# Anaesthesiaye/sound_event_detection_transformer

Hardware: AMD Instinct MI355X
Metric: audio clips/sec training throughput (B=64, 10s@64-mel) (higher is better)
Workload: dtype bf16

## Files before the change

include/sedt_hip.h:

```cpp
#ifndef SEDT_HIP_H
#define SEDT_HIP_H
#include <stddef.h>
#include <stdint.h>

#ifdef __cplusplus
extern "C" {
#endif

#define SEDT_F32 0
#define SEDT_BF16 1
#define SEDT_BF16X3 2
#define SEDT_I16 3

#define SEDT_ACT_NONE 0
#define SEDT_ACT_RELU 1
#define SEDT_ACT_SIGMOID 2

const char* sedt_last_error(void);
int sedt_version(void);

typedef struct SedtIgemm {
  int32_t M, N, K;
  const void* A;
  const void* B;
// ... 64 lines not shown
int sedt_split3(const SedtSplitJob* jobs, int njobs, void* stream);

#define SEDT_MAX_REDUCE_JOBS 40
typedef struct SedtReduceJob {
  const float* slab;
  const float* rowscale;
  float* out;
  const float* colsum_slab;
  float* bias_out;
  int32_t splitk, R, taps, Ci;
  int32_t blk0;
  int32_t cs_splitk;
} SedtReduceJob;
int sedt_multi_wgrad_reduce(const SedtReduceJob* jobs, int njobs, const SedtPrefetch* pf, void* stream);

int sedt_skinny_linear_fwd(const void* x, int64_t ldx, const float* w, const float* bias, void* y, int64_t ldy, int M, int N,
                           int K, int act, int out_f32, int dtype, void* stream);
size_t sedt_skinny_linear_bwd_scratch(int K);
int sedt_skinny_linear_bwd(const float* g, const float* ysaved, int64_t ldg, const float* w, const void* x, int64_t ldx,
                           const void* mask, int64_t ldm, void* gx, int64_t ldo, float* dw, float* db, float* scratch, int M, int N,
                           int K, int act, int accumulate_gx, int dtype, void* stream);

int sedt_colsum(const void* in, int64_t ld, int rows, int cols, int in_f32, int dtype, float* out,
                float* scratch, size_t scratch_bytes, void* stream);
size_t sedt_colsum_scratch(int rows, int cols);
int sedt_dropout_grad(const void* in, int64_t ldi, void* out, int64_t ldo, int rows, int cols, float p,
                      uint32_t seed, const uint32_t* seed_ptr, int dtype, void* stream);
int sedt_add(const void* a, const void* b, void* out, int rows, int cols, int b_mod, int dtype, void* stream);
int sedt_add_n(const void* const* srcs, int n, void* out, int64_t numel, int dtype, void* stream);
int sedt_cast(const void* in, int in_dtype, void* out, int out_dtype, int64_t n, void* stream);
// ... 323 lines not shown
```

sound_event_detection_transformer_amd/csrc/host.cpp:

```cpp
#include <math.h>
#include <stdint.h>
#include <vector>
#include "../../include/sedt_hip.h"

namespace sedt { void set_error(const char* fmt, ...); }

template <typename F>
static void lsa_rows_le_cols(int n, int m, F a, std::vector<int>& row_of_col) {
  const double INF = 1e300;
  std::vector<double> u(n + 1, 0.0), v(m + 1, 0.0), minv(m + 1);
  std::vector<int> p(m + 1, 0), way(m + 1, 0);
  std::vector<char> used(m + 1);
  for (int i = 1; i <= n; ++i) {
    p[0] = i;
    int j0 = 0;
    std::fill(minv.begin(), minv.end(), INF);
    std::fill(used.begin(), used.end(), 0);
    do {
      used[j0] = 1;
      int i0 = p[j0], j1 = 0;
      double delta = INF;
      for (int j = 1; j <= m; ++j) {
        if (used[j]) continue;
        double cur = a(i0 - 1, j - 1) - u[i0] - v[j];
// ... 53 lines not shown
extern "C" int sedt_sizeof(int which) {
  switch (which) {
    case 0: return (int)sizeof(SedtIgemm);
    case 1: return (int)sizeof(SedtReduceJob);
    case 2: return (int)sizeof(SedtSplitJob);
    case 3: return (int)sizeof(SedtPrefetch);
    case 4: return (int)sizeof(SedtCriterion);
    case 5: return (int)sizeof(SedtMatch);
    case 6: return (int)sizeof(SedtChunk);
    case 7: return (int)sizeof(SedtBnJob);
    case 8: return (int)sizeof(SedtPackJob);
    case 9: return (int)sizeof(SedtFragJob);
    case 10: return (int)sizeof(SedtPoolAt);
    case 11: return (int)sizeof(SedtCopyJob);
    case 12: return (int)sizeof(SedtViewAug);
    default: return -1;
  }
}
```

sound_event_detection_transformer_amd/csrc/igemm.hip:

```cpp
#include <stdlib.h>
#include "common.h"

namespace sedt {

template <typename T> struct Cfg;
template <> struct Cfg<float> {
  static constexpr int BK = 32, PITCH = 33, EPC = 4, KSTEP = 2, UK = 1;
};
template <> struct Cfg<bf16_t> {
  static constexpr int BK = 64, PITCH = 72, EPC = 8, KSTEP = 16, UK = 4;
};

struct GatherGeom {
  int Hi, Wi, Ci, Ho, Wo, KH, KW, sh, sw, ph, pw, dh, dw, transposed;
};

__device__ __forceinline__ long gather_pix(const GatherGeom& g, int n, int ho, int wo, int kh, int kw) {
  int hi, wi;
  if (!g.transposed) {
    hi = ho * g.sh - g.ph + kh * g.dh;
    wi = wo * g.sw - g.pw + kw * g.dw;
    if ((unsigned)hi >= (unsigned)g.Hi || (unsigned)wi >= (unsigned)g.Wi) return -1;
  } else {
    int th = ho + g.ph - kh * g.dh, tw = wo + g.pw - kw * g.dw;
// ... 627 lines not shown
    long a, b;
    if (wgrad_lds_envelope(*args, &a, &b) == 0) {
      snprintf(out, cap, "%s", wgrad4_ok(*args) ? "wgrad4_group_kernel" : "wgrad3_group_kernel");
      return 0;
    }
  }
  describe.on = true;
  describe.name[0] = 0;
  const int r = sedt_igemm(args, dtype, nullptr);
  describe.on = false;
  if (r == 0) snprintf(out, cap, "%s", describe.name);
  return r;
}

namespace sedt {
int wgrad3_group_try(const SedtIgemm* jobs, int njobs, hipStream_t st);
bool wgrad4_shape_ok(int M, int N);
int wgrad4_tile_m(int M, int N);
int igemm3_group_try(const SedtIgemm* jobs, int njobs, hipStream_t st);
}

extern "C" int sedt_igemm_group(const SedtIgemm* jobs, int njobs, int dtype, void* stream) {
  SEDT_REQUIRE(jobs && njobs >= 1, "igemm_group: bad arguments");
  for (int i = 0; i < njobs; ++i)
    if (int r = check_rmap(jobs[i])) return r;
  if (dtype == SEDT_BF16 && njobs >= 2) {
    const int r = sedt::igemm3_group_try(jobs, njobs, reinterpret_cast<hipStream_t>(stream));
    if (r >= 0) return r;
  }
  for (int i = 0; i < njobs; ++i)
    if (int r = sedt_igemm(&jobs[i], dtype, stream)) return r;
// ... 5 lines not shown
  SEDT_REQUIRE(jobs && njobs >= 1 && out && cap > 0, "igemm_group_describe: bad arguments");
  out[0] = 0;
  if (dtype != SEDT_BF16 || njobs < 2) return 0;
  describe.on = true;
  describe.name[0] = 0;
  const int r = igemm3_group_try(jobs, njobs, nullptr);
  describe.on = false;
  if (r == 0) snprintf(out, cap, "%s", describe.name);
  return r > 0 ? r : 0;
}

extern "C" int sedt_wgrad_group(const SedtIgemm* jobs, int njobs, int dtype, void* stream) {
  SEDT_REQUIRE(jobs && njobs >= 1, "wgrad_group: bad arguments");
  for (int i = 0; i < njobs; ++i) SEDT_REQUIRE(!jobs[i].rmap, "wgrad_group: a weight-gradient problem takes no residual map (job %d)", i);
  if (dtype == SEDT_BF16) {
    const int r = sedt::wgrad3_group_try(jobs, njobs, reinterpret_cast<hipStream_t>(stream));
    if (r >= 0) return r;
  }
  for (int i = 0; i < njobs; ++i)
    if (int r = sedt_igemm(&jobs[i], dtype, stream)) return r;
  return 0;
}

#include "wgrad3_body.h"
namespace sedt {
int wgrad3_group_build(const SedtIgemm* jobs, int njobs, WgradGroup* g);
extern thread_local const WgradGroup* co_group;
extern thread_local bool co_taken;
}

extern "C" int sedt_igemm_co(const SedtIgemm* main, const SedtIgemm* wjobs, int nw, int dtype, void* stream, int* taken) {
  using namespace sedt;
  SEDT_REQUIRE(main && (nw == 0 || wjobs) && taken, "igemm_co: bad arguments");
  *taken = 0;
  for (int i = 0; i < nw; ++i) SEDT_REQUIRE(!wjobs[i].rmap, "igemm_co: a weight-gradient rider takes no residual map (job %d)", i);
// ... 61 lines not shown
```

sound_event_detection_transformer_amd/csrc/wgrad3.hip:

```cpp
#include <stdlib.h>
#include <algorithm>
#include "wgrad3_body.h"

namespace sedt {

template <int BN>
__global__ __launch_bounds__(256) void wgrad3_kernel(const SedtIgemm p, const unsigned a_bytes, const unsigned b_bytes,
                                                     const int nmajor) {
  wgrad3_body<BN>(p, a_bytes, b_bytes, nmajor, blockIdx.x, blockIdx.y);
}

__global__ __launch_bounds__(256) void wgrad3_group_kernel(const WgradGroup g) { wgrad_group_run(g, blockIdx.x); }

template <int BN>
static int launch_wgrad3(const SedtIgemm& p, unsigned a_bytes, unsigned b_bytes, hipStream_t st) {
  SEDT_DESCRIBE("wgrad3_kernel<%d>", BN);
  constexpr size_t lds = (size_t)2 * (64 * ROWB + 64 * BN * 2);
  static bool attr_set = false;
  auto kern = wgrad3_kernel<BN>;
  if (!attr_set) {
    hipError_t e = hipFuncSetAttribute(reinterpret_cast<const void*>(kern), hipFuncAttributeMaxDynamicSharedMemorySize, (int)lds);
    if (e != hipSuccess) {
      set_error("wgrad3: hipFuncSetAttribute failed: %s", hipGetErrorString(e));
      return 1;
// ... 6 lines not shown
    const char* e = sedt::dev_getenv("SEDT_WGRAD_NMAJOR");
    force = e ? atoi(e) : -1;
  }
  const int nmajor = force >= 0 ? force : (p.N > p.M ? 1 : 0);
  hipLaunchKernelGGL(kern, dim3(nwg, p.splitk > 1 ? p.splitk : 1), dim3(256), lds, st, p, a_bytes, b_bytes, nmajor);
  return check_launch("wgrad3");
}

static bool wgrad3_conv_ok(const SedtIgemm& p) {
  return !(p.conv && ((64 % p.Wo) != 0 || p.Ho * p.Wo < 64 || p.Ho < 64 / p.Wo));
}

int wgrad_lds_envelope(const SedtIgemm& p, long* a_bytes, long* b_bytes);
bool wgrad4_ok(const SedtIgemm& p);
int launch_wgrad4(const SedtIgemm& p, unsigned a_bytes, unsigned b_bytes, hipStream_t st);
int launch_wgrad4_group(WgradGroup& g, hipStream_t st);

int wgrad3_group_try(const SedtIgemm* jobs, int njobs, hipStream_t st) {
  static int on = -1;
  if (on < 0) {
    const char* e = sedt::dev_getenv("SEDT_WGRAD_GROUP");
    on = (e && e[0] == '0') ? 0 : 1;
  }
  if (!on || njobs < 1) return -1;
  long ab[WG_MAXG], bb[WG_MAXG];
  for (int base = 0; base < njobs; base += WG_MAXG) {
    const int n = std::min(WG_MAXG, njobs - base);
    for (int i = 0; i < n; ++i) {
      const SedtIgemm& p = jobs[base + i];
      if (!p.trans || wgrad_lds_envelope(p, &ab[i], &bb[i]) != 0 || !wgrad3_conv_ok(p)) return -1;
    }
  }
  static bool attr_set = false;
  constexpr size_t lds = (size_t)2 * (64 * ROWB + 64 * 64 * 2);
  if (!attr_set) {
    hipError_t e = hipFuncSetAttribute(reinterpret_cast<const void*>(wgrad3_group_kernel), hipFuncAttributeMaxDynamicSharedMemorySize,
                                       (int)lds);
    if (e != hipSuccess) {
      set_error("wgrad3 group: hipFuncSetAttribute failed: %s", hipGetErrorString(e));
      return 1;
    }
    attr_set = true;
  }
  for (int base = 0; base < njobs; base += WG_MAXG) {
    WgradGroup g, gw;
    g.n = gw.n = 0;
    const int n = std::min(WG_MAXG, njobs - base);
    int blk = 0;
    for (int j = 0; j < n; ++j) {
      const SedtIgemm& p = jobs[base + j];
      long a, b;
      wgrad_lds_envelope(p, &a, &b);
      if (wgrad4_ok(p)) {
        const int i = gw.n++;
        gw.p[i] = p;
        gw.a_bytes[i] = (unsigned)a;
        gw.b_bytes[i] = (unsigned)b;
        continue;
      }
      const int i = g.n++;
      g.p[i] = p;
      g.a_bytes[i] = (unsigned)a;
      g.b_bytes[i] = (unsigned)b;
      g.nwg[i] = ((p.N + 63) / 64) * ((p.M + 63) / 64);
      g.nmajor[i] = (p.N > p.M ? 1 : 0) + ((p.splitk >= 8 && p.splitk % 8 == 0) ? 2 : 0);
      g.blk0[i] = blk;
      blk += (g.nwg[i] * (p.splitk > 1 ? p.splitk : 1) + 7) / 8 * 8;
    }
    if (gw.n > 0)
      if (int r = launch_wgrad4_group(gw, st)) return r;
    if (g.n > 0) {
      g.blk0[g.n] = blk;
      hipLaunchKernelGGL(wgrad3_group_kernel, dim3(blk), dim3(256), lds, st, g);
      if (int r = check_launch("wgrad3_group")) return r;
    }
  }
  return 0;
}

int wgrad3_group_build(const SedtIgemm* jobs, int njobs, WgradGroup* g) {
  if (njobs < 1 || njobs > WG_MAXG) return -1;
  g->n = njobs;
  int blk = 0;
  for (int i = 0; i < njobs; ++i) {
    const SedtIgemm& p = jobs[i];
// ... 62 lines not shown
```

sound_event_detection_transformer_amd/csrc/wgrad3_body.h:

```cpp
#pragma once
#include "lds_gemm_common.h"

namespace sedt {

typedef __attribute__((ext_vector_type(4))) short w3_s16x4;
typedef __attribute__((ext_vector_type(8))) short w3_s16x8;
typedef __attribute__((address_space(3))) w3_s16x4 w3_lds_s16x4;

__device__ __forceinline__ int w3_uniform(int v) { return __builtin_amdgcn_readfirstlane(v); }

__device__ __forceinline__ int w3_swz(int row) {
  const int v = (row >> 1) & 7;
  return ((v & 1) << 2) | (v & 2) | (v >> 2);
}

template <int BN, bool CONV>
__device__ __forceinline__ void wgrad3_impl(const SedtIgemm& p, const unsigned a_bytes, const unsigned b_bytes, const int nmajor,
                                            const int bx, const int by) {
  constexpr int BM = 64, BKP = 64;
  constexpr int NI = BN / 64;
  constexpr int A_BYTES = BKP * ROWB;
  constexpr int B_ROWB = BN * 2;
  constexpr int STAGE_BYTES = A_BYTES + BKP * B_ROWB;
  constexpr int GA = 2, GB = BN / 32;
// ... 216 lines not shown
  else wgrad3_impl<BN, false>(p, a_bytes, b_bytes, nmajor, bx, by);
}

constexpr int WG_MAXG = 10;
struct WgradGroup {
  int n;
  int blk0[WG_MAXG + 1];
  int nwg[WG_MAXG];
  int nmajor[WG_MAXG];
  unsigned a_bytes[WG_MAXG], b_bytes[WG_MAXG];
  SedtIgemm p[WG_MAXG];
};

static_assert(sizeof(WgradGroup) <= 3900, "WgradGroup must fit the 4 KB kernel-argument segment");

__device__ __forceinline__ void wgrad_group_run(const WgradGroup& g, const int b) {
  int i = 0;
  while (i + 1 < g.n && b >= g.blk0[i + 1]) ++i;
  const int local = b - g.blk0[i];
  const int nwg = g.nwg[i], sk = g.p[i].splitk > 1 ? g.p[i].splitk : 1;
  if (local >= nwg * sk) return;
  if (g.nmajor[i] >= 2) {
    const int j = local >> 3;
    wgrad3_body<64>(g.p[i], g.a_bytes[i], g.b_bytes[i], g.nmajor[i], j % nwg, (local & 7) + 8 * (j / nwg));
  } else {
    wgrad3_body<64>(g.p[i], g.a_bytes[i], g.b_bytes[i], g.nmajor[i], local % nwg, local / nwg);
  }
}

}
// ... 1 lines not shown
```

sound_event_detection_transformer_amd/csrc/wgrad4.hip:

```cpp
#include <stdlib.h>
#include <algorithm>
#include "wgrad3_body.h"

namespace sedt {

__device__ __forceinline__ int w4_swz(int row) { return (row & 3) << 2; }

template <bool CONV, int S, int NA>
__device__ __forceinline__ void wgrad4_impl(const SedtIgemm& p, const unsigned a_bytes, const unsigned b_bytes, const int nmajor,
                                            const int bx, const int by) {
  constexpr int BM = 128 * NA, BN = 128, BKP = 64, NW = 8;
  constexpr int IMG_ROWB = 256;
  constexpr int IMG_BYTES = BKP * IMG_ROWB;
  constexpr int STAGE_BYTES = (NA + 1) * IMG_BYTES;
  constexpr int B_IMG = NA * IMG_BYTES;
  constexpr int CPR = 16, RPI = 4;
  constexpr int GB = BKP / RPI / NW, GA = NA * GB;
  constexpr int G = GA + GB;
  constexpr int MI = 2 * NA;
  constexpr unsigned OOB = 0x80000000u;
  extern __shared__ __attribute__((aligned(16))) unsigned char smem[];
  const int t = threadIdx.x, lane = t & 63;
  const int wave = w3_uniform(t >> 6);
  const int kgrp = wave >> 2;
  const int wm = ((wave & 3) >> 1) * (32 * MI), wn = (wave & 1) * 64;
// ... 246 lines not shown
        }
  }
  __syncthreads();
  if (kgrp == 1) {
#pragma unroll
    for (int i = 0; i < MI; ++i)
#pragma unroll
      for (int j = 0; j < 2; ++j)
#pragma unroll
        for (int r = 0; r < 16; ++r) {
          const int row = wm + i * 32 + (r & 3) + 8 * (r >> 2) + 4 * fhalf;
          Cs[row * CP + wn + j * 32 + frow] += acc[i][j][r];
        }
  }
  __syncthreads();
  float* out = p.splitk > 1 ? p.slab + (long)by * p.M * p.N : reinterpret_cast<float*>(p.C);
  const long ldo = p.splitk > 1 ? p.N : p.ldc;
#pragma unroll
  for (int c = 0; c < BM * (BN / 4) / (NW * 64); ++c) {
    const int u = t + c * NW * 64;
    const int trow = u / (BN / 4), cc = (u % (BN / 4)) * 4;
    *reinterpret_cast<float4*>(out + (long)(m0 + trow) * ldo + n0 + cc) = *reinterpret_cast<const float4*>(Cs + trow * CP + cc);
  }
}

template <int S>
__device__ __forceinline__ void wgrad4_body(const SedtIgemm& p, const unsigned a_bytes, const unsigned b_bytes, const int nmajor,
                                            const int bx, const int by) {
  if (nmajor & 2) {
    if (p.conv) wgrad4_impl<true, 3, 2>(p, a_bytes, b_bytes, nmajor, bx, by);
    else wgrad4_impl<false, 3, 2>(p, a_bytes, b_bytes, nmajor, bx, by);
    return;
  }
  if (p.conv) wgrad4_impl<true, S, 1>(p, a_bytes, b_bytes, nmajor, bx, by);
  else wgrad4_impl<false, S, 1>(p, a_bytes, b_bytes, nmajor, bx, by);
}

template <int S>
__global__ __launch_bounds__(512) void wgrad4_kernel(const SedtIgemm p, const unsigned a_bytes, const unsigned b_bytes,
                                                     const int nmajor) {
  wgrad4_body<S>(p, a_bytes, b_bytes, nmajor, blockIdx.x, blockIdx.y);
}

template <int S>
__global__ __launch_bounds__(512) void wgrad4_group_kernel(const WgradGroup g) {
  const int b = blockIdx.x;
  int i = 0;
  while (i + 1 < g.n && b >= g.blk0[i + 1]) ++i;
  const int local = b - g.blk0[i];
  const int nwg = g.nwg[i], sk = g.p[i].splitk > 1 ? g.p[i].splitk : 1;
  if (local >= nwg * sk) return;
  wgrad4_body<S>(g.p[i], g.a_bytes[i], g.b_bytes[i], g.nmajor[i], local % nwg, local / nwg);
}

static int wg4_stages() {
  static int s = -1;
  if (s < 0) {
    const char* e = sedt::dev_getenv("SEDT_WGRAD4_STAGES");
    s = (e && atoi(e) == 3) ? 3 : (e && atoi(e) == 4) ? 4 : 3;
  }
  return s;
}
int wgrad4_tile_m(int M, int N) {
  static int bm = -1, min_tiles = 1;
  if (bm < 0) {
    const char* e = sedt::dev_getenv("SEDT_WGRAD4_BM");
    bm = (e && atoi(e) == 128) ? 128 : 256;
// ... 55 lines not shown
  SEDT_DESCRIBE("wgrad4_kernel<%d>", wg4_stages());
  static bool attr_set = false;
  if (!attr_set) {
    if (wg4_attr(wgrad4_kernel<3>, "wgrad4") || wg4_attr(wgrad4_kernel<4>, "wgrad4")) return 1;
    attr_set = true;
  }
  const int bm = wgrad4_tile_m(p.M, p.N);
  const int nwg = (p.N / 128) * (p.M / bm);
  const int nmajor = (p.N > p.M ? 1 : 0) | (bm == 256 ? 2 : 0);
  const dim3 grid(nwg, p.splitk > 1 ? p.splitk : 1);
  if (wg4_stages() == 4) hipLaunchKernelGGL(wgrad4_kernel<4>, grid, dim3(512), wg4_lds(), st, p, a_bytes, b_bytes, nmajor);
  else hipLaunchKernelGGL(wgrad4_kernel<3>, grid, dim3(512), wg4_lds(), st, p, a_bytes, b_bytes, nmajor);
  return check_launch("wgrad4");
}

int launch_wgrad4_group(WgradGroup& g, hipStream_t st) {
  static bool attr_set = false;
  if (!attr_set) {
    if (wg4_attr(wgrad4_group_kernel<3>, "wgrad4 group") || wg4_attr(wgrad4_group_kernel<4>, "wgrad4 group")) return 1;
    attr_set = true;
  }
  int blk = 0;
  for (int i = 0; i < g.n; ++i) {
    const SedtIgemm& p = g.p[i];
    const int bm = wgrad4_tile_m(p.M, p.N);
    g.nwg[i] = (p.N / 128) * (p.M / bm);
    g.nmajor[i] = (p.N > p.M ? 1 : 0) | (bm == 256 ? 2 : 0) | (wg4_cbmajor(p) ? 4 : 0);
    g.blk0[i] = blk;
    blk += (g.nwg[i] * (p.splitk > 1 ? p.splitk : 1) + 7) / 8 * 8;
  }
  g.blk0[g.n] = blk;
  if (wg4_stages() == 4) hipLaunchKernelGGL(wgrad4_group_kernel<4>, dim3(blk), dim3(512), wg4_lds(), st, g);
  else hipLaunchKernelGGL(wgrad4_group_kernel<3>, dim3(blk), dim3(512), wg4_lds(), st, g);
  return check_launch("wgrad4_group");
}

}
```

sound_event_detection_transformer_amd/lib.py:

```python
import ctypes as C
import os

import torch

HERE = os.path.dirname(os.path.abspath(__file__))
LIB_PATH = os.path.join(HERE, 'libsedt_hip.so')
if os.environ.get('SEDT_LIB_AB') and os.environ.get('SEDT_DEV') == '1':
    LIB_PATH = os.environ['SEDT_LIB_AB']

F32, BF16 = 0, 1
BF16X3 = 2
I16 = 3
GEMM_X3 = False


def gemm_dtype(dtype):
    return BF16X3 if (dtype == F32 and GEMM_X3) else dtype
ACT_NONE, ACT_RELU, ACT_SIGMOID = 0, 1, 2
TORCH_DTYPE = {F32: torch.float32, BF16: torch.bfloat16}


class SedtIgemm(C.Structure):
    _fields_ = [
        ('M', C.c_int32), ('N', C.c_int32), ('K', C.c_int32),
# ... 12 lines not shown
        ('splitk', C.c_int32), ('slab', C.c_void_p),
        ('tile_m', C.c_int32), ('tile_n', C.c_int32),
        ('colsum_out', C.c_void_p),
        ('bits_out', C.c_void_p), ('ldbits', C.c_int64), ('mask_bits', C.c_int32), ('f32ep', C.c_int32),
        ('omap', C.c_int32), ('o_Hi', C.c_int32), ('o_Wi', C.c_int32), ('o_sh', C.c_int32), ('o_sw', C.c_int32), ('o_h0', C.c_int32),
        ('o_w0', C.c_int32), ('btap_on', C.c_int32), ('btap', C.c_int32 * 8), ('split_out', C.c_void_p), ('awrap', C.c_int32), ('rmap', C.c_int32), ('bfrag', C.c_void_p),
    ]


class SedtReduceJob(C.Structure):
    _fields_ = [('slab', C.c_void_p), ('rowscale', C.c_void_p), ('out', C.c_void_p), ('colsum_slab', C.c_void_p),
                ('bias_out', C.c_void_p), ('splitk', C.c_int32), ('R', C.c_int32), ('taps', C.c_int32), ('Ci', C.c_int32),
                ('blk0', C.c_int32), ('cs_splitk', C.c_int32)]


CRIT_MAXL = 8


class SedtCriterion(C.Structure):
    _fields_ = [(n, C.c_void_p) for n in ('logits', 'boxes', 'at', 'tc', 'coef', 'wbox', 'tbox', 'gt_weak', 'tgt_len',
                                           'num_boxes', 'empty_weight', 'dlogits', 'dboxes', 'dboxes2', 'dat', 'out')] + \
               [(n, C.c_int32) for n in ('L', 'B', 'ns', 'Q', 'C', 'n_lab', 'Bat')] + \
               [('layer_of', C.c_int32 * CRIT_MAXL), ('w_ce', C.c_float * CRIT_MAXL), ('w_bbox', C.c_float * CRIT_MAXL),
                ('w_giou', C.c_float * CRIT_MAXL), ('w_weak', C.c_float), ('fl', C.c_int32), ('alpha_fl', C.c_float),
                ('gamma_fl', C.c_float), ('nonfinite', C.c_void_p), ('split', C.c_void_p), ('Qs', C.c_int32), ('q0', C.c_int32),
                ('total', C.c_void_p), ('at_p', C.c_void_p), ('dat_p', C.c_void_p), ('w_weak_p', C.c_float), ('wp_all', C.c_int32),
                ('Bp', C.c_int32)]


class SedtPoolAt(C.Structure):
# ... 36 lines not shown
    for i, t in enumerate(ts):
        a.ptr[i], a.bytes[i] = t.data_ptr(), t.numel() * t.element_size()
    return C.byref(a)


MAX_REDUCE_JOBS = 40
_vp, _i, _i64, _f, _d, _u32, _sz = C.c_void_p, C.c_int, C.c_int64, C.c_float, C.c_double, C.c_uint32, C.c_size_t

SIGNATURES = {
    'sedt_last_error': (C.c_char_p, []),
    'sedt_version': (_i, []),
    'sedt_sizeof': (_i, [_i]),
    'sedt_igemm': (_i, [C.POINTER(SedtIgemm), _i, _vp]),
    'sedt_igemm_group': (_i, [C.POINTER(SedtIgemm), _i, _i, _vp]),
    'sedt_wgrad_group': (_i, [C.POINTER(SedtIgemm), _i, _i, _vp]),
    'sedt_igemm_co': (_i, [C.POINTER(SedtIgemm), C.POINTER(SedtIgemm), _i, _i, _vp, C.POINTER(C.c_int)]),
    'sedt_igemm_splitk': (_i, [_i, _i, _i, _i]),
    'sedt_igemm_describe': (_i, [C.POINTER(SedtIgemm), _i, _i, C.c_char_p, _i]),
    'sedt_igemm_group_describe': (_i, [C.POINTER(SedtIgemm), _i, _i, C.c_char_p, _i]),
    'sedt_wgrad_reduce': (_i, [_vp, _i, _i, _i, _i, _vp, _vp, _vp]),
    'sedt_wgrad_reduce_bias': (_i, [_vp, _i, _i, _i, _i, _vp, _vp, _vp, _vp, _vp]),
    'sedt_split3': (_i, [C.POINTER(SedtSplitJob), _i, _vp]),
    'sedt_copy2d': (_i, [C.POINTER(SedtCopyJob), _i, _vp]),
    'sedt_multi_wgrad_reduce': (_i, [C.POINTER(SedtReduceJob), _i, C.POINTER(SedtPrefetch), _vp]),
    'sedt_skinny_linear_fwd': (_i, [_vp, _i64, _vp, _vp, _vp, _i64, _i, _i, _i, _i, _i, _i, _vp]),
    'sedt_skinny_linear_bwd_scratch': (_sz, [_i]),
    'sedt_skinny_linear_bwd': (_i, [_vp, _vp, _i64, _vp, _vp, _i64, _vp, _i64, _vp, _i64, _vp, _vp, _vp, _i, _i, _i, _i, _i, _i, _vp]),
    'sedt_colsum': (_i, [_vp, _i64, _i, _i, _i, _i, _vp, _vp, _sz, _vp]),
    'sedt_colsum_scratch': (_sz, [_i, _i]),
    'sedt_dropout_grad': (_i, [_vp, _i64, _vp, _i64, _i, _i, _f, _u32, _vp, _i, _vp]),
# ... 138 lines not shown
```

sound_event_detection_transformer_amd/ops.py:

```python
import ctypes as C

import os
import numpy as np
import torch

from . import lib as L
from .lib import F32, BF16, ACT_NONE, ACT_RELU, ACT_SIGMOID, TORCH_DTYPE, p as _p


class ConvGeom(object):
    __slots__ = ('Hi', 'Wi', 'Ci', 'Ho', 'Wo', 'Co', 'KH', 'KW', 'sh', 'sw', 'ph', 'pw', 'dh', 'dw')

    def __init__(self, Hi, Wi, Ci, Co, k=1, stride=1, pad=0, dil=1):
        self.Hi, self.Wi, self.Ci, self.Co = Hi, Wi, Ci, Co
        self.KH = self.KW = k
        self.sh = self.sw = stride
        self.ph = self.pw = pad
        self.dh = self.dw = dil
        self.Ho = (Hi + 2 * pad - dil * (k - 1) - 1) // stride + 1
        self.Wo = (Wi + 2 * pad - dil * (k - 1) - 1) // stride + 1

    @property
    def taps(self):
        return self.KH * self.KW
# ... 575 lines not shown
        L.LAUNCH_LOG['proj_dgrad:%dx%dx%d' % (M, g.Ci, g.Co)] += 1
    igemm(dtype, M, g.Ci, g.Co, dy, dy.stride(0), wb, g.Co, side, side.stride(0))
    return side, dict(ldr=side.stride(0), res_map=(g.Hi, g.Wi, g.sh, g.sw))


def _fused_bias_ok(dtype, dy, x, g):
    return (dtype == BF16 and L.load() is not None and g.Co % 8 == 0 and (g.taps * g.Ci) % 8 == 0 and dy.stride(0) % 8 == 0
            and x.stride(0) % 8 == 0 and dy.data_ptr() % 16 == 0 and x.data_ptr() % 16 == 0 and g.Ci % 8 == 0)


class ReduceBatch(object):

    def __init__(self, shared=False):
        self.jobs, self.keep, self.deferred, self.operands = [], [], [], []
        self.group, self.group_dtype = [], None
        self.shared = shared
        self.expect = []

    def add_gemm(self, dtype, args, shape, code=None):
        self.group.append((args, shape, L.gemm_dtype(dtype) if code is None else code))
        self.group_dtype = dtype

    def _launch_group(self):
        if not self.group:
            return
        lib = L.load()
        if PROFILE is not None:
            for a, shape, code in self.group:
                L.check(lib.sedt_igemm(C.byref(a), code, L.stream_ptr()), 'sedt_igemm')
                PROFILE.append((a, code, shape, (list(self.keep), list(self.operands)), 'wgrad_group'))
        else:
            i = 0
            while i < len(self.group):
                j = i
                while j < len(self.group) and self.group[j][2] == self.group[i][2]:
                    j += 1
                arr = (L.SedtIgemm * (j - i))(*[g[0] for g in self.group[i:j]])
                L.check(lib.sedt_wgrad_group(arr, j - i, self.group[i][2], L.stream_ptr()), 'wgrad_group')
                i = j
        self.group = []

    def defer(self, body, operands):
        self.deferred.append(body)
        self.operands.extend(t for t in operands if t is not None)

    def add(self, slab, sk, R, taps, Ci, rowscale, out, cs, bias_out, cs_splitk=0):
        j = L.SedtReduceJob()
        j.slab, j.out, j.splitk, j.R, j.taps, j.Ci = slab.data_ptr(), out.data_ptr(), sk, R, taps, Ci
        j.cs_splitk = cs_splitk
        j.rowscale = rowscale.data_ptr() if rowscale is not None else None
        j.colsum_slab = cs.data_ptr() if cs is not None else None
        j.bias_out = bias_out.data_ptr() if (cs is not None and bias_out is not None) else None
        self.jobs.append(j)
        self.keep.append((slab, cs, rowscale, None, None) if self.shared else (slab, cs, rowscale, out, bias_out))
        if len(self.jobs) == L.MAX_REDUCE_JOBS and not _co['on'] and not self.shared:
# ... 34 lines not shown
                POOL.push(self.group, BF16, self.jobs, [k[:3] for k in self.keep], self.operands)
                self.group, self.jobs, self.keep, self.operands = [], [], [], []
                return
        if self.deferred:
            with runtime.side(*self.operands):
                for body in self.deferred:
                    body()
                self._launch_group()
                self._launch()
            self.deferred, self.operands = [], []
        else:
            self._launch_group()
            self._launch()


DEFER_LAYER_WGRADS = _dev_env('SEDT_DEFER_LAYER_WGRADS', '1') != '0'
_defer = {'on': False}


class defer_layer_wgrads(object):

    def __init__(self, enable=True):
        self.enable = bool(enable) and DEFER_LAYER_WGRADS

    def __enter__(self):
        self.prev = _defer['on']
        _defer['on'] = self.enable
        return self

    def __exit__(self, *exc):
# ... 92 lines not shown
            slab = torch.empty((3 * sk3, Mo, No), device=dy.device, dtype=torch.float32)
            cs = torch.empty((2 * sk3, Mo), device=dy.device, dtype=torch.float32) if bias_out is not None else None
            a1 = igemm_args(2 * Mo, No, Kp, dy3, 2 * Mo, x3, 2 * g.Ci, slab, No, trans=1, conv=conv, out_f32=1, splitk=sk3, slab=slab,
                            colsum_out=cs)
            x3lo, slab2 = x3[:, g.Ci:2 * g.Ci], slab[2 * sk3:]
            a2 = igemm_args(Mo, No, Kp, dy3, 2 * Mo, x3lo, 2 * g.Ci, slab2, No, trans=1, conv=conv, out_f32=1, splitk=sk3, slab=slab2)
            tb = batch if batch is not None else ReduceBatch()
            tb.add_gemm(dtype, a1, (2 * Mo, No, Kp, 1, 0 if conv is None else 1), code=BF16)
            tb.add_gemm(dtype, a2, (Mo, No, Kp, 1, 0 if conv is None else 1), code=BF16)
            tb.add(slab, 3 * sk3, Mo, g.taps, g.Ci, rowscale, out, cs, bias_out, cs_splitk=2 * sk3)
            tb.keep.append((dy3, x3, None, None, None))
            if batch is None:
                tb._launch_group()
                tb._launch()
            return
        slab = torch.empty((sk, Mo, No), device=dy.device, dtype=torch.float32)
        fused = bias_out is not None and _fused_bias_ok(dtype, dy, x, g)
        cs = torch.empty((sk, Mo), device=dy.device, dtype=torch.float32) if fused else None
        if batch is not None:
            batch.add_gemm(dtype, igemm_args(Mo, No, Kp, dy, dy.stride(0), x, x.stride(0), slab, No, trans=1, conv=conv,
                                             out_f32=1, splitk=sk, slab=slab, colsum_out=cs),
                           (Mo, No, Kp, 1, 0 if conv is None else 1))
            batch.add(slab, sk, Mo, g.taps, g.Ci, rowscale, out, cs, bias_out if fused else None)
        else:
            igemm(dtype, Mo, No, Kp, dy, dy.stride(0), x, x.stride(0), slab, No, trans=1, conv=conv, out_f32=1, splitk=sk,
                  slab=slab, colsum_out=cs)
            L.check(lib.sedt_wgrad_reduce_bias(_p(slab), sk, Mo, g.taps, g.Ci, _p(rowscale), _p(out), _p(cs),
                                               _p(bias_out) if fused else None, L.stream_ptr()), 'wgrad_reduce')
        if bias_out is not None and not fused:
            colsum(dtype, dy, out=bias_out)

    if batch is not None:
# ... 841 lines not shown
```

Measured before the change: 12830.

## Fuse split-K reduction and weight-gradient finish into wgrad4 group kernel epilogue

```diff
diff --git a/include/sedt_hip.h b/include/sedt_hip.h
--- a/include/sedt_hip.h
+++ b/include/sedt_hip.h
@@ -102,6 +102,15 @@
 } SedtReduceJob;
 int sedt_multi_wgrad_reduce(const SedtReduceJob* jobs, int njobs, const SedtPrefetch* pf, void* stream);
 
+#define SEDT_FINISH_COUNTERS 65536
+typedef struct SedtWgradFinish {
+  float* out;
+  const float* rowscale;
+  int32_t taps, Ci;
+} SedtWgradFinish;
+int sedt_wgrad_group_finish(const SedtIgemm* jobs, const SedtWgradFinish* fin, int njobs, int dtype, const SedtPrefetch* pf, void* stream);
+int sedt_wgrad_group_finishes(const SedtIgemm* job, const SedtWgradFinish* fin, int dtype);
+
 int sedt_skinny_linear_fwd(const void* x, int64_t ldx, const float* w, const float* bias, void* y, int64_t ldy, int M, int N,
                            int K, int act, int out_f32, int dtype, void* stream);
 size_t sedt_skinny_linear_bwd_scratch(int K);
diff --git a/sound_event_detection_transformer_amd/csrc/host.cpp b/sound_event_detection_transformer_amd/csrc/host.cpp
--- a/sound_event_detection_transformer_amd/csrc/host.cpp
+++ b/sound_event_detection_transformer_amd/csrc/host.cpp
@@ -91,6 +91,7 @@
     case 10: return (int)sizeof(SedtPoolAt);
     case 11: return (int)sizeof(SedtCopyJob);
     case 12: return (int)sizeof(SedtViewAug);
+    case 13: return (int)sizeof(SedtWgradFinish);
     default: return -1;
   }
 }
diff --git a/sound_event_detection_transformer_amd/csrc/igemm.hip b/sound_event_detection_transformer_amd/csrc/igemm.hip
--- a/sound_event_detection_transformer_amd/csrc/igemm.hip
+++ b/sound_event_detection_transformer_amd/csrc/igemm.hip
@@ -665,7 +665,9 @@
 }
 
 namespace sedt {
-int wgrad3_group_try(const SedtIgemm* jobs, int njobs, hipStream_t st);
+int wgrad3_group_try(const SedtIgemm* jobs, int njobs, hipStream_t st, const SedtWgradFinish* fin, const SedtPrefetch* pf);
+bool wgrad_group_finishes(const SedtIgemm& p, const SedtWgradFinish& f);
+int wgrad4_finish_one(const SedtIgemm& p, const SedtWgradFinish& f, hipStream_t st);
 bool wgrad4_shape_ok(int M, int N);
 int wgrad4_tile_m(int M, int N);
 int igemm3_group_try(const SedtIgemm* jobs, int njobs, hipStream_t st);
@@ -701,11 +703,32 @@
   SEDT_REQUIRE(jobs && njobs >= 1, "wgrad_group: bad arguments");
   for (int i = 0; i < njobs; ++i) SEDT_REQUIRE(!jobs[i].rmap, "wgrad_group: a weight-gradient problem takes no residual map (job %d)", i);
   if (dtype == SEDT_BF16) {
-    const int r = sedt::wgrad3_group_try(jobs, njobs, reinterpret_cast<hipStream_t>(stream));
+    const int r = sedt::wgrad3_group_try(jobs, njobs, reinterpret_cast<hipStream_t>(stream), nullptr, nullptr);
     if (r >= 0) return r;
   }
   for (int i = 0; i < njobs; ++i)
     if (int r = sedt_igemm(&jobs[i], dtype, stream)) return r;
+  return 0;
+}
+
+extern "C" int sedt_wgrad_group_finishes(const SedtIgemm* job, const SedtWgradFinish* fin, int dtype) {
+  return (job && fin && dtype == SEDT_BF16 && !job->rmap && sedt::wgrad_group_finishes(*job, *fin)) ? 1 : 0;
+}
+
+extern "C" int sedt_wgrad_group_finish(const SedtIgemm* jobs, const SedtWgradFinish* fin, int njobs, int dtype, const SedtPrefetch* pf,
+                                       void* stream) {
+  SEDT_REQUIRE(jobs && fin && njobs >= 1, "wgrad_group_finish: bad arguments");
+  for (int i = 0; i < njobs; ++i) SEDT_REQUIRE(!jobs[i].rmap, "wgrad_group_finish: a weight-gradient problem takes no residual map (job %d)", i);
+  hipStream_t st = reinterpret_cast<hipStream_t>(stream);
+  if (dtype == SEDT_BF16) {
+    const int r = sedt::wgrad3_group_try(jobs, njobs, st, fin, pf);
+    if (r >= 0) return r;
+  }
+  for (int i = 0; i < njobs; ++i) {
+    if (sedt_wgrad_group_finishes(&jobs[i], &fin[i], dtype)) {
+      if (int r = sedt::wgrad4_finish_one(jobs[i], fin[i], st)) return r;
+    } else if (int r = sedt_igemm(&jobs[i], dtype, stream)) return r;
+  }
   return 0;
 }
 
diff --git a/sound_event_detection_transformer_amd/csrc/wgrad3.hip b/sound_event_detection_transformer_amd/csrc/wgrad3.hip
--- a/sound_event_detection_transformer_amd/csrc/wgrad3.hip
+++ b/sound_event_detection_transformer_amd/csrc/wgrad3.hip
@@ -44,15 +44,36 @@
 int wgrad_lds_envelope(const SedtIgemm& p, long* a_bytes, long* b_bytes);
 bool wgrad4_ok(const SedtIgemm& p);
 int launch_wgrad4(const SedtIgemm& p, unsigned a_bytes, unsigned b_bytes, hipStream_t st);
-int launch_wgrad4_group(WgradGroup& g, hipStream_t st);
-
-int wgrad3_group_try(const SedtIgemm* jobs, int njobs, hipStream_t st) {
+int launch_wgrad4_group(WgradGroup& g, const SedtWgradFinish* fin, const SedtPrefetch* pf, hipStream_t st);
+bool wgrad4_finishes(const SedtIgemm& p, const SedtWgradFinish& f);
+
+static bool wgrad_group_on() {
   static int on = -1;
   if (on < 0) {
     const char* e = sedt::dev_getenv("SEDT_WGRAD_GROUP");
     on = (e && e[0] == '0') ? 0 : 1;
   }
-  if (!on || njobs < 1) return -1;
+  return on == 1;
+}
+
+bool wgrad_group_finishes(const SedtIgemm& p, const SedtWgradFinish& f) {
+  long a, b;
+  return wgrad_group_on() && p.trans && wgrad_lds_envelope(p, &a, &b) == 0 && wgrad3_conv_ok(p) && wgrad4_finishes(p, f);
+}
+
+int wgrad4_finish_one(const SedtIgemm& p, const SedtWgradFinish& f, hipStream_t st) {
+  WgradGroup gw;
+  long a, b;
+  wgrad_lds_envelope(p, &a, &b);
+  gw.n = 1;
+  gw.p[0] = p;
+  gw.a_bytes[0] = (unsigned)a;
+  gw.b_bytes[0] = (unsigned)b;
+  return launch_wgrad4_group(gw, &f, nullptr, st);
+}
+
+int wgrad3_group_try(const SedtIgemm* jobs, int njobs, hipStream_t st, const SedtWgradFinish* fin, const SedtPrefetch* pf) {
+  if (!wgrad_group_on() || njobs < 1) return -1;
   long ab[WG_MAXG], bb[WG_MAXG];
   for (int base = 0; base < njobs; base += WG_MAXG) {
     const int n = std::min(WG_MAXG, njobs - base);
@@ -74,6 +95,7 @@
   }
   for (int base = 0; base < njobs; base += WG_MAXG) {
     WgradGroup g, gw;
+    SedtWgradFinish fw[WG_MAXG] = {};
     g.n = gw.n = 0;
     const int n = std::min(WG_MAXG, njobs - base);
     int blk = 0;
@@ -86,6 +108,7 @@
         gw.p[i] = p;
         gw.a_bytes[i] = (unsigned)a;
         gw.b_bytes[i] = (unsigned)b;
+        if (fin && wgrad4_finishes(p, fin[base + j])) fw[i] = fin[base + j];
         continue;
       }
       const int i = g.n++;
@@ -98,7 +121,7 @@
       blk += (g.nwg[i] * (p.splitk > 1 ? p.splitk : 1) + 7) / 8 * 8;
     }
     if (gw.n > 0)
-      if (int r = launch_wgrad4_group(gw, st)) return r;
+      if (int r = launch_wgrad4_group(gw, fin ? fw : nullptr, base + WG_MAXG >= njobs ? pf : nullptr, st)) return r;
     if (g.n > 0) {
       g.blk0[g.n] = blk;
       hipLaunchKernelGGL(wgrad3_group_kernel, dim3(blk), dim3(256), lds, st, g);
diff --git a/sound_event_detection_transformer_amd/csrc/wgrad3_body.h b/sound_event_detection_transformer_amd/csrc/wgrad3_body.h
--- a/sound_event_detection_transformer_amd/csrc/wgrad3_body.h
+++ b/sound_event_detection_transformer_amd/csrc/wgrad3_body.h
@@ -254,6 +254,15 @@
 
 static_assert(sizeof(WgradGroup) <= 3900, "WgradGroup must fit the 4 KB kernel-argument segment");
 
+struct Wg4Finish {
+  float* out[WG_MAXG];
+  const float* rowscale[WG_MAXG];
+  unsigned* cnt[WG_MAXG];
+  int taps[WG_MAXG], Ci[WG_MAXG];
+  const uint32_t* pf[3];
+  int pf_lines[3];
+};
+
 __device__ __forceinline__ void wgrad_group_run(const WgradGroup& g, const int b) {
   int i = 0;
   while (i + 1 < g.n && b >= g.blk0[i + 1]) ++i;
diff --git a/sound_event_detection_transformer_amd/csrc/wgrad4.hip b/sound_event_detection_transformer_amd/csrc/wgrad4.hip
--- a/sound_event_detection_transformer_amd/csrc/wgrad4.hip
+++ b/sound_event_detection_transformer_amd/csrc/wgrad4.hip
@@ -1,14 +1,22 @@
 #include <stdlib.h>
 #include <algorithm>
+#include <mutex>
 #include "wgrad3_body.h"
 
 namespace sedt {
 
 __device__ __forceinline__ int w4_swz(int row) { return (row & 3) << 2; }
+
+struct W4Fin {
+  float* out;
+  const float* rowscale;
+  unsigned* cnt;
+  int taps, Ci;
+};
 
 template <bool CONV, int S, int NA>
 __device__ __forceinline__ void wgrad4_impl(const SedtIgemm& p, const unsigned a_bytes, const unsigned b_bytes, const int nmajor,
-                                            const int bx, const int by) {
+                                            const int bx, const int by, const W4Fin f) {
   constexpr int BM = 128 * NA, BN = 128, BKP = 64, NW = 8;
   constexpr int IMG_ROWB = 256;
   constexpr int IMG_BYTES = BKP * IMG_ROWB;
@@ -285,43 +293,128 @@
         }
   }
   __syncthreads();
-  float* out = p.splitk > 1 ? p.slab + (long)by * p.M * p.N : reinterpret_cast<float*>(p.C);
-  const long ldo = p.splitk > 1 ? p.N : p.ldc;
-#pragma unroll
-  for (int c = 0; c < BM * (BN / 4) / (NW * 64); ++c) {
-    const int u = t + c * NW * 64;
-    const int trow = u / (BN / 4), cc = (u % (BN / 4)) * 4;
-    *reinterpret_cast<float4*>(out + (long)(m0 + trow) * ldo + n0 + cc) = *reinterpret_cast<const float4*>(Cs + trow * CP + cc);
+  constexpr int NC = BM * (BN / 4) / (NW * 64);
+  if (f.out == nullptr || p.splitk > 1) {
+    float* out = p.splitk > 1 ? p.slab + (long)by * p.M * p.N : reinterpret_cast<float*>(p.C);
+    const long ldo = p.splitk > 1 ? p.N : p.ldc;
+#pragma unroll
+    for (int c = 0; c < NC; ++c) {
+      const int u = t + c * NW * 64;
+      const int trow = u / (BN / 4), cc = (u % (BN / 4)) * 4;
+      *reinterpret_cast<float4*>(out + (long)(m0 + trow) * ldo + n0 + cc) = *reinterpret_cast<const float4*>(Cs + trow * CP + cc);
+    }
+    if (f.out == nullptr) return;
+  }
+
+  if (p.splitk > 1) {
+    static_assert((size_t)BM * CP * 4 + 16 <= (size_t)S * STAGE_BYTES, "the last-arriver word sits behind the epilogue tile");
+    volatile unsigned* last_flag = reinterpret_cast<volatile unsigned*>(smem + (size_t)BM * CP * 4);
+    asm volatile("s_waitcnt vmcnt(0)" ::: "memory");
+    __syncthreads();
+    if (t == 0) {
+      __builtin_amdgcn_fence(__ATOMIC_RELEASE, "agent");
+      asm volatile("s_waitcnt vmcnt(0)" ::: "memory");
+      unsigned* cnt = f.cnt + bx;
+      const unsigned ticket = __hip_atomic_fetch_add(cnt, 1u, __ATOMIC_RELAXED, __HIP_MEMORY_SCOPE_AGENT);
+      const unsigned last = ticket == (unsigned)p.splitk - 1u ? 1u : 0u;
+      if (last) {
+        __builtin_amdgcn_fence(__ATOMIC_ACQUIRE, "agent");
+        asm volatile("s_waitcnt vmcnt(0)" ::: "memory");
+        __hip_atomic_store(cnt, 0u, __ATOMIC_RELAXED, __HIP_MEMORY_SCOPE_AGENT);
+      }
+      *last_flag = last;
+    }
+    __syncthreads();
+    if (*last_flag == 0u) return;
+    float4 sum[NC];
+    for (int z = 0; z < p.splitk; ++z) {
+      float4 v[NC];
+      if (z == by) {
+#pragma unroll
+        for (int c = 0; c < NC; ++c) {
+          const int u = t + c * NW * 64;
+          v[c] = *reinterpret_cast<const float4*>(Cs + (u / (BN / 4)) * CP + (u % (BN / 4)) * 4);
+        }
+      } else {
+        const float* sl = p.slab + (long)z * p.M * p.N + (long)m0 * p.N + n0;
+#pragma unroll
+        for (int c = 0; c < NC; ++c) {
+          const int u = t + c * NW * 64;
+          v[c] = *reinterpret_cast<const float4*>(sl + (long)(u / (BN / 4)) * p.N + (u % (BN / 4)) * 4);
+        }
+      }
+#pragma unroll
+      for (int c = 0; c < NC; ++c) {
+        if (z == 0) sum[c] = v[c];
+        else { sum[c].x += v[c].x; sum[c].y += v[c].y; sum[c].z += v[c].z; sum[c].w += v[c].w; }
+      }
+    }
+#pragma unroll
+    for (int c = 0; c < NC; ++c) {
+      const int u = t + c * NW * 64;
+      *reinterpret_cast<float4*>(Cs + (u / (BN / 4)) * CP + (u % (BN / 4)) * 4) = sum[c];
+    }
+    __syncthreads();
+  }
+  if (f.taps == 1) {
+#pragma unroll
+    for (int c = 0; c < NC; ++c) {
+      const int u = t + c * NW * 64;
+      const int trow = u / (BN / 4), cc = (u % (BN / 4)) * 4;
+      float4 v = *reinterpret_cast<const float4*>(Cs + trow * CP + cc);
+      if (f.rowscale) {
+        const float sc = f.rowscale[m0 + trow];
+        v.x *= sc; v.y *= sc; v.z *= sc; v.w *= sc;
+      }
+      *reinterpret_cast<float4*>(f.out + (long)(m0 + trow) * p.N + n0 + cc) = v;
+    }
+  } else {
+    for (int c = 0; c < BM * BN / (NW * 64); ++c) {
+      const int u = t + c * NW * 64;
+      const int trow = u / BN, col = u % BN;
+      const int n = n0 + col, tap = n / f.Ci, ch = n - tap * f.Ci;
+      float v = Cs[trow * CP + col];
+      if (f.rowscale) v *= f.rowscale[m0 + trow];
+      f.out[((long)(m0 + trow) * f.Ci + ch) * f.taps + tap] = v;
+    }
   }
 }
 
 template <int S>
 __device__ __forceinline__ void wgrad4_body(const SedtIgemm& p, const unsigned a_bytes, const unsigned b_bytes, const int nmajor,
-                                            const int bx, const int by) {
+                                            const int bx, const int by, const W4Fin f) {
   if (nmajor & 2) {
-    if (p.conv) wgrad4_impl<true, 3, 2>(p, a_bytes, b_bytes, nmajor, bx, by);
-    else wgrad4_impl<false, 3, 2>(p, a_bytes, b_bytes, nmajor, bx, by);
+    if (p.conv) wgrad4_impl<true, 3, 2>(p, a_bytes, b_bytes, nmajor, bx, by, f);
+    else wgrad4_impl<false, 3, 2>(p, a_bytes, b_bytes, nmajor, bx, by, f);
     return;
   }
-  if (p.conv) wgrad4_impl<true, S, 1>(p, a_bytes, b_bytes, nmajor, bx, by);
-  else wgrad4_impl<false, S, 1>(p, a_bytes, b_bytes, nmajor, bx, by);
+  if (p.conv) wgrad4_impl<true, S, 1>(p, a_bytes, b_bytes, nmajor, bx, by, f);
+  else wgrad4_impl<false, S, 1>(p, a_bytes, b_bytes, nmajor, bx, by, f);
 }
 
 template <int S>
 __global__ __launch_bounds__(512) void wgrad4_kernel(const SedtIgemm p, const unsigned a_bytes, const unsigned b_bytes,
                                                      const int nmajor) {
-  wgrad4_body<S>(p, a_bytes, b_bytes, nmajor, blockIdx.x, blockIdx.y);
+  wgrad4_body<S>(p, a_bytes, b_bytes, nmajor, blockIdx.x, blockIdx.y, W4Fin{nullptr, nullptr, nullptr, 1, 0});
 }
 
 template <int S>
-__global__ __launch_bounds__(512) void wgrad4_group_kernel(const WgradGroup g) {
-  const int b = blockIdx.x;
+__global__ __launch_bounds__(512) void wgrad4_group_kernel(const WgradGroup g, const Wg4Finish fin) {
+  const int b = blockIdx.x, nblk = g.blk0[g.n];
+  uint32_t touched = 0;
+  if (b + 256 >= nblk && fin.pf_lines[0] + fin.pf_lines[1] + fin.pf_lines[2] > 0) {
+    const int slot = (nblk - 1 - b) >> 3, nslots = min(32, max(1, nblk >> 3));
+    for (int r = 0; r < 3; ++r)
+      for (int j = slot * 512 + (int)threadIdx.x; j < fin.pf_lines[r]; j += nslots * 512) touched ^= fin.pf[r][(long)j * 32];
+  }
   int i = 0;
   while (i + 1 < g.n && b >= g.blk0[i + 1]) ++i;
   const int local = b - g.blk0[i];
   const int nwg = g.nwg[i], sk = g.p[i].splitk > 1 ? g.p[i].splitk : 1;
-  if (local >= nwg * sk) return;
-  wgrad4_body<S>(g.p[i], g.a_bytes[i], g.b_bytes[i], g.nmajor[i], local % nwg, local / nwg);
+  if (local < nwg * sk)
+    wgrad4_body<S>(g.p[i], g.a_bytes[i], g.b_bytes[i], g.nmajor[i], local % nwg, local / nwg,
+                   W4Fin{fin.out[i], fin.rowscale[i], fin.cnt[i], fin.taps[i], fin.Ci[i]});
+  if (touched == 0x9e3779b9u && g.n < 0) g.p[0].slab[0] = 1.f;
 }
 
 static int wg4_stages() {
@@ -407,13 +500,58 @@
   return check_launch("wgrad4");
 }
 
-int launch_wgrad4_group(WgradGroup& g, hipStream_t st) {
+static std::mutex fin_mutex;
+static unsigned* fin_buf[16] = {nullptr};
+static unsigned fin_cursor[16] = {0};
+static unsigned* fin_take(int need, hipStream_t st) {
+  int dev = 0;
+  if (hipGetDevice(&dev) != hipSuccess || dev < 0 || dev >= 16) {
+    set_error("wgrad4 group: finishing counters support devices 0..15");
+    return nullptr;
+  }
+  std::lock_guard<std::mutex> lock(fin_mutex);
+  if (!fin_buf[dev]) {
+    hipStreamCaptureStatus cs = hipStreamCaptureStatusNone;
+    if (st && hipStreamIsCapturing(st, &cs) == hipSuccess && cs != hipStreamCaptureStatusNone) {
+      set_error("wgrad4 group: the first finishing launch on a device allocates its counters and must run outside a stream capture");
+      return nullptr;
+    }
+    unsigned* b = nullptr;
+    if (hipMalloc(&b, SEDT_FINISH_COUNTERS * sizeof(unsigned)) != hipSuccess || hipMemset(b, 0, SEDT_FINISH_COUNTERS * sizeof(unsigned)) != hipSuccess ||
+        hipDeviceSynchronize() != hipSuccess) {
+      set_error("wgrad4 group: cannot allocate the finishing counters");
+      return nullptr;
+    }
+    fin_buf[dev] = b;
+  }
+  if (fin_cursor[dev] + (unsigned)need > SEDT_FINISH_COUNTERS) fin_cursor[dev] = 0;
+  unsigned* r = fin_buf[dev] + fin_cursor[dev];
+  fin_cursor[dev] += (unsigned)need;
+  return r;
+}
+
+bool wgrad4_finishes(const SedtIgemm& p, const SedtWgradFinish& f) {
+  static int on = -1;
+  if (on < 0) {
+    const char* e = sedt::dev_getenv("SEDT_WGRAD_FINISH");
+    on = (e && e[0] == '0') ? 0 : 1;
+  }
+  if (!on || !f.out || (reinterpret_cast<uintptr_t>(f.out) & 15) || !wgrad4_ok(p) || p.colsum_out) return false;
+  if (f.taps < 1 || f.Ci < 4 || (f.Ci & 3) || (long)f.taps * f.Ci != p.N) return false;
+  if (p.conv ? !(p.KH * p.KW == f.taps && p.Ci == f.Ci) : f.taps != 1) return false;
+  if (p.splitk <= 1 && (p.C != f.out || p.ldc != p.N)) return false;
+  const long nwg = (long)(p.N / 128) * (p.M / wgrad4_tile_m(p.M, p.N));
+  return nwg <= SEDT_FINISH_COUNTERS / (2 * WG_MAXG);
+}
+
+int launch_wgrad4_group(WgradGroup& g, const SedtWgradFinish* fin, const SedtPrefetch* pf, hipStream_t st) {
   static bool attr_set = false;
   if (!attr_set) {
     if (wg4_attr(wgrad4_group_kernel<3>, "wgrad4 group") || wg4_attr(wgrad4_group_kernel<4>, "wgrad4 group")) return 1;
     attr_set = true;
   }
-  int blk = 0;
+  Wg4Finish x = {};
+  int blk = 0, ncnt = 0;
   for (int i = 0; i < g.n; ++i) {
     const SedtIgemm& p = g.p[i];
     const int bm = wgrad4_tile_m(p.M, p.N);
@@ -421,10 +559,32 @@
     g.nmajor[i] = (p.N > p.M ? 1 : 0) | (bm == 256 ? 2 : 0) | (wg4_cbmajor(p) ? 4 : 0);
     g.blk0[i] = blk;
     blk += (g.nwg[i] * (p.splitk > 1 ? p.splitk : 1) + 7) / 8 * 8;
+    x.taps[i] = 1;
+    if (fin && fin[i].out) {
+      x.out[i] = fin[i].out;
+      x.rowscale[i] = fin[i].rowscale;
+      x.taps[i] = fin[i].taps;
+      x.Ci[i] = fin[i].Ci;
+      if (p.splitk > 1) ncnt += g.nwg[i];
+    }
   }
   g.blk0[g.n] = blk;
-  if (wg4_stages() == 4) hipLaunchKernelGGL(wgrad4_group_kernel<4>, dim3(blk), dim3(512), wg4_lds(), st, g);
-  else hipLaunchKernelGGL(wgrad4_group_kernel<3>, dim3(blk), dim3(512), wg4_lds(), st, g);
+  if (ncnt > 0) {
+    unsigned* c = fin_take(ncnt, st);
+    if (!c) return 1;
+    for (int i = 0; i < g.n; ++i)
+      if (x.out[i] && g.p[i].splitk > 1) {
+        x.cnt[i] = c;
+        c += g.nwg[i];
+      }
+  }
+  if (pf)
+    for (int r = 0; r < 3; ++r) {
+      x.pf[r] = reinterpret_cast<const uint32_t*>(pf->ptr[r]);
+      x.pf_lines[r] = pf->ptr[r] ? (int)std::min<size_t>(pf->bytes[r] / 128, (size_t)1 << 24) : 0;
+    }
+  if (wg4_stages() == 4) hipLaunchKernelGGL(wgrad4_group_kernel<4>, dim3(blk), dim3(512), wg4_lds(), st, g, x);
+  else hipLaunchKernelGGL(wgrad4_group_kernel<3>, dim3(blk), dim3(512), wg4_lds(), st, g, x);
   return check_launch("wgrad4_group");
 }
 
diff --git a/sound_event_detection_transformer_amd/lib.py b/sound_event_detection_transformer_amd/lib.py
--- a/sound_event_detection_transformer_amd/lib.py
+++ b/sound_event_detection_transformer_amd/lib.py
@@ -50,6 +50,10 @@
                 ('blk0', C.c_int32), ('cs_splitk', C.c_int32)]
 
 
+class SedtWgradFinish(C.Structure):
+    _fields_ = [('out', C.c_void_p), ('rowscale', C.c_void_p), ('taps', C.c_int32), ('Ci', C.c_int32)]
+
+
 CRIT_MAXL = 8
 
 
@@ -116,6 +120,8 @@
     'sedt_igemm': (_i, [C.POINTER(SedtIgemm), _i, _vp]),
     'sedt_igemm_group': (_i, [C.POINTER(SedtIgemm), _i, _i, _vp]),
     'sedt_wgrad_group': (_i, [C.POINTER(SedtIgemm), _i, _i, _vp]),
+    'sedt_wgrad_group_finish': (_i, [C.POINTER(SedtIgemm), C.POINTER(SedtWgradFinish), _i, _i, C.POINTER(SedtPrefetch), _vp]),
+    'sedt_wgrad_group_finishes': (_i, [C.POINTER(SedtIgemm), C.POINTER(SedtWgradFinish), _i]),
     'sedt_igemm_co': (_i, [C.POINTER(SedtIgemm), C.POINTER(SedtIgemm), _i, _i, _vp, C.POINTER(C.c_int)]),
     'sedt_igemm_splitk': (_i, [_i, _i, _i, _i]),
     'sedt_igemm_describe': (_i, [C.POINTER(SedtIgemm), _i, _i, C.c_char_p, _i]),
diff --git a/sound_event_detection_transformer_amd/ops.py b/sound_event_detection_transformer_amd/ops.py
--- a/sound_event_detection_transformer_amd/ops.py
+++ b/sound_event_detection_transformer_amd/ops.py
@@ -613,12 +613,16 @@
     def __init__(self, shared=False):
         self.jobs, self.keep, self.deferred, self.operands = [], [], [], []
         self.group, self.group_dtype = [], None
+        self.fin = {}
         self.shared = shared
         self.expect = []
 
-    def add_gemm(self, dtype, args, shape, code=None):
+    def add_gemm(self, dtype, args, shape, code=None, fin=None, keep=None):
         self.group.append((args, shape, L.gemm_dtype(dtype) if code is None else code))
         self.group_dtype = dtype
+        if fin is not None:
+            self.fin[id(args)] = fin
+            self.keep.append(keep)
 
     def _launch_group(self):
         if not self.group:
@@ -635,9 +639,17 @@
                 while j < len(self.group) and self.group[j][2] == self.group[i][2]:
                     j += 1
                 arr = (L.SedtIgemm * (j - i))(*[g[0] for g in self.group[i:j]])
-                L.check(lib.sedt_wgrad_group(arr, j - i, self.group[i][2], L.stream_ptr()), 'wgrad_group')
+                fins = [self.fin.get(id(g[0])) for g in self.group[i:j]]
+                if any(f is not None for f in fins):
+                    farr = (L.SedtWgradFinish * (j - i))(*[f if f is not None else L.SedtWgradFinish() for f in fins])
+                    pf = None
+                    if self.prefetch is not None and RED_PREFETCH and not self.jobs and j == len(self.group):
+                        pf = L.prefetch_arg(self.prefetch)
+                    L.check(lib.sedt_wgrad_group_finish(arr, farr, j - i, self.group[i][2], pf, L.stream_ptr()), 'wgrad_group')
+                else:
+                    L.check(lib.sedt_wgrad_group(arr, j - i, self.group[i][2], L.stream_ptr()), 'wgrad_group')
                 i = j
-        self.group = []
+        self.group, self.fin = [], {}
 
     def defer(self, body, operands):
         self.deferred.append(body)
@@ -702,6 +714,8 @@
             self._launch()
 
 
+WGRAD_FINISH = _dev_env('SEDT_WGRAD_FINISH', '1') != '0'
+
 DEFER_LAYER_WGRADS = _dev_env('SEDT_DEFER_LAYER_WGRADS', '1') != '0'
 _defer = {'on': False}
 
@@ -824,8 +838,24 @@
                 tb._launch_group()
                 tb._launch()
             return
-        slab = torch.empty((sk, Mo, No), device=dy.device, dtype=torch.float32)
         fused = bias_out is not None and _fused_bias_ok(dtype, dy, x, g)
+        slab = None
+        if (WGRAD_FINISH and batch is not None and dtype == BF16 and not fused and not _co['on'] and PROFILE is None
+                and out.dtype == torch.float32 and out.is_contiguous() and out.data_ptr() % 16 == 0):
+            fin = L.SedtWgradFinish()
+            fin.out, fin.taps, fin.Ci = out.data_ptr(), g.taps, g.Ci
+            fin.rowscale = rowscale.data_ptr() if rowscale is not None else None
+            slab = torch.empty((sk, Mo, No), device=dy.device, dtype=torch.float32) if sk > 1 else None
+            a = igemm_args(Mo, No, Kp, dy, dy.stride(0), x, x.stride(0), slab if sk > 1 else out, No, trans=1, conv=conv, out_f32=1,
+                           splitk=sk, slab=slab)
+            if lib.sedt_wgrad_group_finishes(C.byref(a), C.byref(fin), dtype):
+                batch.add_gemm(dtype, a, (Mo, No, Kp, 1, 0 if conv is None else 1), fin=fin,
+                               keep=(slab, None, rowscale, None if batch.shared else out, None))
+                if bias_out is not None:
+                    colsum(dtype, dy, out=bias_out)
+                return
+        if slab is None:
+            slab = torch.empty((sk, Mo, No), device=dy.device, dtype=torch.float32)
         cs = torch.empty((sk, Mo), device=dy.device, dtype=torch.float32) if fused else None
         if batch is not None:
             batch.add_gemm(dtype, igemm_args(Mo, No, Kp, dy, dy.stride(0), x, x.stride(0), slab, No, trans=1, conv=conv,
```

Result: slower. 12500 (-2.6%).
